# jpedro1992/gym-loadbalancing

Measured on AMD Instinct MI355X. Metric: env-steps/sec (whole node) at 1M envs, 1/2/4/8 GPUs; % HBM roofline, higher is better.
Workload: dtype f64

## Files before the change

### gym-loadbalancing_amd/csrc/lbk8s_lean.h

```cpp
#pragma once

#include "lbk8s_rollout.h"

namespace lbk {

typedef __amdgpu_buffer_rsrc_t Rsrc;
typedef uint32_t u32x2 __attribute__((ext_vector_type(2)));
typedef uint32_t u32x4 __attribute__((ext_vector_type(4)));

__device__ __forceinline__ Rsrc rsrc_of(const void* base) {
    return __builtin_amdgcn_make_buffer_rsrc(const_cast<void*>(base), (short)0, -1, 0x00020000);
}
constexpr int BUF_NT = 2;

#define LB_GUARD_S(...) asm volatile("" : "+s"(__VA_ARGS__))
#define LB_GUARD_V(...) asm volatile("" : "+v"(__VA_ARGS__))

__device__ __forceinline__ double buf_ld_f64(Rsrc r, uint32_t off) {
    return __builtin_bit_cast(double, __builtin_amdgcn_raw_buffer_load_b64(r, off, 0, 0));
}
__device__ __forceinline__ uint4 buf_ld_u128(Rsrc r, uint32_t off) {
    const u32x4 v = __builtin_amdgcn_raw_buffer_load_b128(r, off, 0, 0);
    return make_uint4(v.x, v.y, v.z, v.w);
}
template <int AUX>
__device__ __forceinline__ void buf_st_f4(float4 v, Rsrc r, uint32_t voff) {
    const u32x4 d{__float_as_uint(v.x), __float_as_uint(v.y), __float_as_uint(v.z), __float_as_uint(v.w)};
    __builtin_amdgcn_raw_buffer_store_b128(d, r, voff, 0, AUX);
}

__device__ __forceinline__ U4 draw_o(const Params& p, int64_t env, uint32_t episode, uint32_t slot, uint32_t dom) {
    uint32_t k0 = p.key0, k1 = p.key1;
    LB_GUARD_S(k0);
    LB_GUARD_S(k1);
    const uint64_t gid = (uint64_t)(p.env_id_offset + env);
    uint32_t c0 = (uint32_t)gid, hi = (uint32_t)(gid >> 32) << 8;
    LB_GUARD_V(c0);
    LB_GUARD_V(hi);
    return philox(c0, episode, slot, dom | hi, k0, k1);
}
__device__ __forceinline__ void draw2_o(const Params& p, int64_t env, uint32_t episode, uint32_t slot, uint32_t dom_a,
                                        uint32_t dom_b, U4& a, U4& b) {
    uint32_t k0 = p.key0, k1 = p.key1;
    LB_GUARD_S(k0);
    LB_GUARD_S(k1);
    const uint64_t gid = (uint64_t)(p.env_id_offset + env);
    uint32_t c0 = (uint32_t)gid, hi = (uint32_t)(gid >> 32) << 8;
    LB_GUARD_V(c0);
    LB_GUARD_V(hi);
    uint32_t a0 = c0, a1 = episode, a2 = slot, a3 = dom_a | hi;
    uint32_t b0 = c0, b1 = episode, b2 = slot, b3 = dom_b | hi;
#pragma unroll
    for (int i = 0; i < LB_PHILOX_ROUNDS; ++i) {
        const uint64_t pa0 = (uint64_t)0xD2511F53u * a0, pa1 = (uint64_t)0xCD9E8D57u * a2;
        const uint64_t pb0 = (uint64_t)0xD2511F53u * b0, pb1 = (uint64_t)0xCD9E8D57u * b2;
        const uint32_t na0 = (uint32_t)(pa1 >> 32) ^ a1 ^ k0, na2 = (uint32_t)(pa0 >> 32) ^ a3 ^ k1;
        const uint32_t nb0 = (uint32_t)(pb1 >> 32) ^ b1 ^ k0, nb2 = (uint32_t)(pb0 >> 32) ^ b3 ^ k1;
        a0 = na0; a1 = (uint32_t)pa1; a2 = na2; a3 = (uint32_t)pa0;
        b0 = nb0; b1 = (uint32_t)pb1; b2 = nb2; b3 = (uint32_t)pb0;
        k0 += 0x9E3779B9u;
        k1 += 0xBB67AE85u;
    }
    a = {a0, a1, a2, a3};
    b = {b0, b1, b2, b3};
}

template <int KIND>
__device__ __forceinline__ int lean_policy(const Params& p, int64_t env, const TEnv& tv, const uint32_t (&em)[TPE_E],
                                           const uint32_t (&ed)[TPE_E]) {
    if constexpr (KIND == LB_POLICY_RANDOM) {
        const U4 w = draw_o(p, env, (uint32_t)(tv.acc3 >> 32), (uint32_t)tv.s.step, D_ACT);
        return (int)bounded(w.x, (uint32_t)p.A);
    }
    return tpe_policy<KIND>(p, env, tv, em, ed);
}

__device__ __forceinline__ int topo_bf(uint64_t topo, int a, int b) {
    const int i = a < b ? a : b, j = a < b ? b : a;
    const int val = (int)((topo >> (9 * ((i * (7 - i)) / 2 + j - i - 1))) & 0x1FF);
    return a == b ? 1 : val;
}

struct LPrepL {
    uint32_t arz;
    uint32_t jm;
    double sel_lat, sel_cpu, next_lat, next_cpu, arr;
    float dt;
};

template <int ET, int RT, int RF>
__device__ __forceinline__ double lean_apply_l(const Params& p, const LPrepL& pr, LEnv& v,
                                               const uint32_t (&em)[TPE_E], uint32_t (&ed)[TPE_E], uint32_t* me) {
    constexpr int E = ET;
    const int rf = RF >= 0 ? RF : p.reward_fn;
    const int a = (int)(pr.arz & 0xFFu);
    const bool accept = a < E, reject = a == E;
    const int ai = accept ? a : 0;
    if (!((v.s1 >> S1_RD) & 1)) v.s1 |= 1u << S1_BAD;
    const int oA = (int)((pr.arz >> 14) & 7u);
    const int jA = (int)(pr.jm & 0x3FFu), Mn = (int)((pr.jm >> 10) & 0x3FFu), MA = (int)(pr.jm >> 20);
    const int jn = jA < CMAX ? jA + 1 : CMAX;
    double reward;
    if (accept) {
        int cnt = 0;
#pragma unroll
        for (int e = 0; e < TPE_E; ++e)
            if (e < E && e != ai && ed_j(ed[e]) <= jA) ++cnt;
        const int rz = (int)((v.s1 >> S1_RZ) & 3), zA = (int)((pr.arz >> 17) & 3u);
        const int tl = topo_bf(v.topo, rz, zA);
        const uint32_t gnum = (uint32_t)(v.acc2 >> 32) + (uint32_t)(2 * (2 * cnt - (E - 1)));
        v.acc2 = ((uint64_t)gnum << 32) | (uint32_t)((uint32_t)v.acc2 + (uint32_t)tl);
        v.acc3 += (uint64_t)node_cost((int)((pr.arz >> 19) & 7u));
        v.s0 += 1u << 16;
        if (rz == zA) v.s1 += 1;
        xsum_add(v.sum_lat, v.sum_cpu, v.sum_hi, pr.sel_lat, pr.sel_cpu, tl, rz != zA);
        const uint32_t edA_new = ((oA == ai ? (uint32_t)Mn : (uint32_t)MA) << 20) |
                                 ((uint32_t)Mn << 10) | (uint32_t)jn;
#pragma unroll
        for (int e = 0; e < TPE_E; ++e) {
            const uint32_t edo = e == oA ? (ed[e] & ~(0x3FFu << 20)) | ((uint32_t)Mn << 20) : ed[e];
            ed[e] = e == ai ? edA_new : edo;
        }
        img_sel(me, ai, (float)pr.next_cpu, (float)pr.next_lat);
        v.s1 &= ~(1u << S1_PEN);
        reward = rf == LB_REWARD_NAIVE ? 1.0 : accept_reward(p, pr.sel_lat, tl, pr.sel_cpu, v.acc2, (int)(v.s0 >> 16));
        v.last_r = reward;
    } else if (reject) {
        v.s1 |= 1u << S1_PEN;
        reward = rf == LB_REWARD_LATENCY ? -1000.0 : -1.0;
        v.last_r = reward;
    } else {
        reward = rf == LB_REWARD_NAIVE ? (((v.s1 >> S1_PEN) & 1) ? -1.0 : 1.0) : v.last_r;
    }
    v.total += reward;
    v.dt = pr.dt;
    v.t = pr.arr;
    v.s1 = (v.s1 & ~((3u << S1_RZ) | (7u << S1_THR))) | (((pr.arz >> 12) & 3u) << S1_RZ) |
           (((pr.arz >> 8) & 7u) << S1_THR);
    img_request(me, v, em, E);
    return reward;
}

constexpr uint32_t LREC_LAT0 = 96;
constexpr uint32_t LREC_ACC = 12;
__device__ __forceinline__ float4 u4f(double a, uint64_t b) {
    const uint64_t x = (uint64_t)__double_as_longlong(a);
    return make_float4(__uint_as_float((uint32_t)x), __uint_as_float((uint32_t)(x >> 32)), __uint_as_float((uint32_t)b),
                       __uint_as_float((uint32_t)(b >> 32)));
}
__device__ __forceinline__ float4 u4f(uint64_t a, uint64_t b) {
    return make_float4(__uint_as_float((uint32_t)a), __uint_as_float((uint32_t)(a >> 32)), __uint_as_float((uint32_t)b),
                       __uint_as_float((uint32_t)(b >> 32)));
}

template <int W>
__device__ __forceinline__ void lean_write_record(const Params& p, int64_t env, uint32_t episode, int lane) {
    static_assert(W == 8, "eight lanes per record (the node packing covers nodes < 24 = 3 x 8)");
    uint64_t zc = 0, nz0 = 0, nz1 = 0;
    uint32_t hp01 = 0, hp2 = 0;
    for (int w = 0; w < p.NZW; ++w) {
        uint64_t word = 0;
        int j = 0;
        for (int n = 32 * w + lane; n < 32 * (w + 1) && n < p.N; n += W, ++j) {
            int ty, zo, cpu;
            node_draw<false>(p, env, episode, n, ty, zo, cpu);
            zc += (uint64_t)node_cpu_int(ty) << (16 * zo);
            word |= (uint64_t)zo << (2 * (n & 31));
            const uint32_t hp = (uint32_t)ty | ((uint32_t)zo << 3) | ((uint32_t)cpu << 5);
            if (w == 0 && j == 0) hp01 |= hp;
            if (w == 0 && j == 1) hp01 |= hp << 16;
            if (w == 0 && j == 2) hp2 = hp;
        }
        word = slice_or64<W>(word);
        if (w == 0) nz0 = word;
        if (w == 1) nz1 = word;
    }
    zc = slice_sum64<W>(zc);
    double lat0 = 0.0;
    int node = 0;
    if (lane < p.E) {
        const U4 d = draw(p, env, episode, (uint32_t)lane, D_EP);
        lat0 = 1.0 + 99.0 * u53(d.x, d.y);
        node = (int)bounded(d.z, 24);
    }
    int owner = lane;
    for (int e2 = 0; e2 < p.E; ++e2) {
        const int nd2 = (int)shfl_u32<W>((uint32_t)node, e2);
        if (nd2 == node && e2 < owner) owner = e2;
    }
    const uint32_t ha = shfl_u32<W>(hp01, node & 7), hb = shfl_u32<W>(hp2, node & 7);
    const uint32_t hp = (node >> 3) == 0 ? (ha & 0xFFFFu) : (node >> 3) == 1 ? (ha >> 16) : hb;
    uint32_t* out = reinterpret_cast<uint32_t*>(p.rec + env * (RO_REC_BYTES / 16));
    if (lane < p.E) {
        const int ty = (int)(hp & 7u), zo = (int)((hp >> 3) & 3u), cpu = (int)((hp >> 5) & 0x7Fu);
        const uint64_t lb = (uint64_t)__double_as_longlong(lat0);
        *reinterpret_cast<uint2*>(out + 24 + 2 * lane) = make_uint2((uint32_t)lb, (uint32_t)(lb >> 32));
        out[lane] = em_pack(zo, owner, ty, cpu, node);
    }
    const int role = lane;
    const U4 w = draw(p, env, episode, role == 4 ? 1u : 0u,
                      role == 2 ? D_REQ_I : (role == 3 || role == 4) ? D_TOPO : D_REQ_X);
    const double e = role == 1 ? std_exp(w.z, w.w) : std_exp(w.x, w.y);
    const double x1 = p.inv_rate * shfl_f64<W>(e, 0), x2 = p.call * shfl_f64<W>(e, 1);
    const int r = (int)bounded(shfl_u32<W>(w.x, 2), 7), n = (int)bounded(shfl_u32<W>(w.y, 2), (uint32_t)p.N);
    const uint32_t a0 = shfl_u32<W>(w.x, 3), a1 = shfl_u32<W>(w.y, 3), a2 = shfl_u32<W>(w.z, 3),
                   a3 = shfl_u32<W>(w.w, 3), b0 = shfl_u32<W>(w.x, 4), b1 = shfl_u32<W>(w.y, 4);
    if (lane == 0) {
        const uint64_t topo = (uint64_t)(1 + bounded(a0, 499)) | ((uint64_t)(1 + bounded(a1, 499)) << 9) |
                              ((uint64_t)(1 + bounded(a2, 499)) << 18) | ((uint64_t)(1 + bounded(a3, 499)) << 27) |
                              ((uint64_t)(1 + bounded(b0, 499)) << 36) | ((uint64_t)(1 + bounded(b1, 499)) << 45);
        const int rz = (int)(((n < 32 ? nz0 : nz1) >> (2 * (n & 31))) & 3);
        const uint64_t wd[6] = {topo, zc, nz0, nz1, (uint64_t)__double_as_longlong(x1),
                                (uint64_t)__double_as_longlong(x2)};
#pragma unroll
        for (int j = 0; j < 6; ++j)
            *reinterpret_cast<uint2*>(out + 8 + 2 * j) = make_uint2((uint32_t)wd[j], (uint32_t)(wd[j] >> 32));
        out[20] = (uint32_t)((r + 6) % 7) | ((uint32_t)rz << 8);
    }
}

template <int ET, int RT, int NG>
__device__ __forceinline__ void lean_restart_group(const Params& p, const LDims<ET, RT>& d, uint32_t* wimg,
                                                   uint64_t grp, int lane, bool mine, LEnv& v,
                                                   uint32_t (&em)[TPE_E], uint32_t (&ed)[TPE_E], uint32_t* me) {
    if (mine) {
        const uint4* q = reinterpret_cast<const uint4*>(me);
        const uint4 s0 = q[2], s1 = q[3], s2 = q[4];
        const uint32_t s3 = me[20];
        v.topo = (uint64_t)s0.x | ((uint64_t)s0.y << 32);
        v.zcap = (uint64_t)s0.z | ((uint64_t)s0.w << 32);
        v.nz0 = (uint64_t)s1.x | ((uint64_t)s1.y << 32);
        v.nz1 = (uint64_t)s1.z | ((uint64_t)s1.w << 32);
        const uint32_t episode = (uint32_t)(v.acc3 >> 32) + 1;
        v.acc3 = (uint64_t)episode << 32;
        v.acc2 = 0;
        v.sum_lat = 0;
        v.sum_cpu = 0;
        v.sum_hi = 0;
        v.total = 0.0;
        v.last_r = p.init_last_r;
        v.s0 = 0;
        v.s1 = (v.s1 & (1u << S1_BAD)) | (1u << S1_RD) | ((s3 & 7u) << S1_THR) | (((s3 >> 8) & 3u) << S1_RZ);
        const double x1 = __longlong_as_double((long long)((uint64_t)s2.x | ((uint64_t)s2.y << 32)));
        const double x2 = __longlong_as_double((long long)((uint64_t)s2.z | ((uint64_t)s2.w << 32)));
        const double arrival = v.t + x1;
        const double departure = arrival + x2;
        v.dt = (float)(departure - arrival);
        v.t = arrival;
    }
    const int e = lane & 7, g = lane >> 3;
    int el = -1;
    {
        uint64_t m = grp;
#pragma unroll
        for (int i = 0; i < NG; ++i) {
            const int b = m ? (int)__builtin_ctzll(m) : -1;
            if (g == i) el = b;
            m &= m - 1;
        }
    }
    const bool helper = el >= 0 && e < ET;
    uint32_t* ri = wimg + (el < 0 ? 0 : el) * IMG_W;
    uint32_t mw = 0, l0lo = 0, l0hi = 0, zlo = 0, zhi = 0;
    if (helper) {
        mw = ri[e];
        l0lo = ri[24 + 2 * e];
        l0hi = ri[25 + 2 * e];
        zlo = ri[10];
        zhi = ri[11];
    }
    wave_lds_sync();
    if (helper) {
        const double l0 = __longlong_as_double((long long)((uint64_t)l0lo | ((uint64_t)l0hi << 32)));
        const int z = em_zone(mw);
        const uint64_t zcap = (uint64_t)zlo | ((uint64_t)zhi << 32);
        *reinterpret_cast<uint4*>(ri + 4 * e) =
            make_uint4(img_zc(z, zcap_val(zcap, z)), 0u, __float_as_uint((float)em_c0(mw)), __float_as_uint((float)l0));
        ri[32 + e] = lem_make(mw, l0);
    }
    wave_lds_sync();
    if (mine) {
        const uint4 a = *reinterpret_cast<const uint4*>(me + 32), b = *reinterpret_cast<const uint4*>(me + 36);
        const uint32_t lw[8] = {a.x, a.y, a.z, a.w, b.x, b.y, b.z, b.w};
#pragma unroll
        for (int i = 0; i < TPE_E; ++i) {
            em[i] = i < ET ? lw[i] : 0u;
            ed[i] = 0u;
        }
        *reinterpret_cast<uint4*>(me + 4 * d.E) = make_uint4(IMG_ZC_REJECT, F32_M1, F32_M1, F32_M1);
        img_request(me, v, em, d.E);
    }
}

template <int NJ>
__device__ __forceinline__ int rec_fetch_env(uint64_t m, int lane, int& chunk) {
    static_assert(NJ <= 6, "64 lanes: 6 records of 10 chunks");
    const int i = lane / 10;
    chunk = lane - 10 * i;
    int el = -1;
#pragma unroll
    for (int j = 0; j < NJ; ++j) {
        const int b = m ? (int)__builtin_ctzll(m) : -1;
        if (i == j) el = b;
        m &= m - 1;
    }
    return el;
}
constexpr int REC_FETCH_MAX = 6;

struct Acc {
    double total;
    uint64_t acc2, acc3, sum_lat, sum_cpu;
    uint32_t sum_hi, s0, s1;
};
template <int ET>
__device__ __forceinline__ void stats_row_lds(uint32_t* me, const Acc& a) {
    static_assert(LB_ST_RETURN == 0 && LB_ST_LENGTH == 1 && LB_ST_ACCEPTED == 2 && LB_ST_SUM_LATENCY == 3 &&
                      LB_ST_SUM_TOPOLOGY == 4 && LB_ST_SUM_TOPOLOGY_UPDATED == 5 && LB_ST_SUM_COST == 6 &&
                      LB_ST_SUM_CPU == 7 && LB_ST_INTRA == 8 && LB_ST_INTER == 9 && LB_ST_GINI == 10 &&
                      LB_ST_EPISODE == 11 && LB_ST_SUM_LATENCY_REM == 12 && LB_ST_SUM_CPU_REM == 13 &&
                      LB_ST_SUM_TOPOLOGY_UPDATED_D == 14 && LB_ST_K == 16,
                  "ep_stats column order");
    const Scal s = sc_unpack((uint64_t)a.s0 | ((uint64_t)a.s1 << 32));
    const uint32_t sum_topo = (uint32_t)a.acc2;
    auto put = [&](int i, double x, double y) {
        const uint64_t lo = (uint64_t)__double_as_longlong(x), hi = (uint64_t)__double_as_longlong(y);
        *reinterpret_cast<uint4*>(me + 4 * i) = make_uint4((uint32_t)lo, (uint32_t)(lo >> 32), (uint32_t)hi, (uint32_t)(hi >> 32));
    };
    double ls, lr, cs, cr;
    put(0, a.total, (double)s.step);
    xsum_pair(a.sum_lat, a.sum_hi & 0x7Fu, ls, lr);
    put(1, (double)s.acc, ls);
    put(2, (double)sum_topo, (double)s.intra + 1.7 * (double)(sum_topo - (uint32_t)s.intra));
    xsum_pair(a.sum_cpu, (a.sum_hi >> XH_CPU) & 0x1Fu, cs, cr);
    put(3, (double)(uint32_t)a.acc3, cs);
    put(4, (double)s.intra, (double)(s.acc - s.intra));
    put(5, gini_of(a.acc2, s.acc, ET), (double)(uint32_t)(a.acc3 >> 32));
    put(6, lr, cr);
    put(7, (double)((int32_t)a.sum_hi >> XH_D), 0.0);
}
__device__ __forceinline__ int nth_env8(uint64_t m, int i) {
    int el = -1;
#pragma unroll
    for (int j = 0; j < 8; ++j) {
        const int b = m ? (int)__builtin_ctzll(m) : -1;
        if (i == j) el = b;
        m &= m - 1;
    }
    return el;
}
__device__ __forceinline__ u32x4 lds_u4(const uint32_t* a) {
    const uint4 q = *reinterpret_cast<const uint4*>(a);
    return u32x4{q.x, q.y, q.z, q.w};
}

template <int P>
__device__ __forceinline__ int term_group_env(uint64_t m, int lane) {
    constexpr int G = 64 / P;
    const int g = lane / P;
    int el = -1;
#pragma unroll
    for (int i = 0; i < G; ++i) {
        const int b = m ? (int)__builtin_ctzll(m) : -1;
        if (g == i) el = b;
        m &= m - 1;
    }
    return el;
}
template <int P>
__device__ __forceinline__ uint64_t drop_low(uint64_t m) {
#pragma unroll
    for (int i = 0; i < 64 / P; ++i) m &= m - 1;
    return m;
}
__device__ __forceinline__ float4 term_piece(const uint32_t* wimg, int el, int pc) {
    const char* base = reinterpret_cast<const char*>(wimg) + el * (IMG_W * 4);
    const uint4 A = *reinterpret_cast<const uint4*>(base + 16 * (pc >> 1));
    const uint4 S = *reinterpret_cast<const uint4*>(base + 4 * IMG_S);
    return img_piece(A, S, (pc & 1) != 0);
}

template <int P>
__device__ __forceinline__ float4 lean_piece(const uint32_t* wimg, int lane, int it, bool h) {
    constexpr uint32_t MAG = (65536u + P - 1) / P;
    static_assert(P % 2 == 0 && 64u * P * (MAG * P - 65536u) < 65536u, "piece / P by multiply, exact below 64 P");
    const uint32_t e = ((uint32_t)lane * MAG + (uint32_t)it * (64u * MAG)) >> 16;
    const char* b = reinterpret_cast<const char*>(wimg);
    const uint4 A = *reinterpret_cast<const uint4*>(b + e * (uint32_t)(IMG_W * 4 - 8 * P) + 16u * (uint32_t)(lane >> 1) +
                                                    512u * (uint32_t)it);
    const uint4 S = *reinterpret_cast<const uint4*>(b + e * (uint32_t)(IMG_W * 4) + 4u * IMG_S);
    return img_piece(A, S, h);
}

#ifdef LB_TIMELINE
#include "../../tools/diag/lbk8s_lean_timeline.h"
#else
#define LB_LTL(k, i) ((void)0)
#define LB_LTL_HDR(slot) ((void)0)
#define LB_LTL_HWID() ((void)0)
#endif

constexpr int LEAN_NB = 64;

constexpr uint32_t SD_BASE = 3 * 64 * 4, SD_BUF = 64 * 20, SD_X2 = 64 * 8, SD_W = 64 * 16;
__device__ __forceinline__ double* sd_x1(uint32_t* sst, int b) {
    return reinterpret_cast<double*>(reinterpret_cast<char*>(sst) + SD_BASE + b * SD_BUF);
}
__device__ __forceinline__ double* sd_x2(uint32_t* sst, int b) { return sd_x1(sst, b) + 64; }
__device__ __forceinline__ uint32_t* sd_w(uint32_t* sst, int b) {
    return reinterpret_cast<uint32_t*>(reinterpret_cast<char*>(sst) + SD_BASE + b * SD_BUF + SD_W);
}
template <int KIND>
__device__ __forceinline__ void split_draws(const Params& p, int64_t env, uint32_t ep, uint32_t cs, uint32_t* sst,
                                            int b, int lane) {
    uint32_t a = 0;
    if constexpr (KIND == LB_POLICY_RANDOM) a = bounded(draw_o(p, env, ep, cs, D_ACT).x, (uint32_t)p.A);
    U4 wx, wi;
    draw2_o(p, env, ep, cs + 1, D_REQ_X, D_REQ_I, wx, wi);
    sd_x1(sst, b)[lane] = p.inv_rate * std_exp(wx.x, wx.y);
    sd_x2(sst, b)[lane] = p.call * std_exp(wx.z, wx.w);
    sd_w(sst, b)[lane] = a | (bounded(wi.x, 7) << 8) | (bounded(wi.y, (uint32_t)p.N) << 16);
}

template <int P, bool ACT, int CW, int KIND>
__device__ __forceinline__ void lean_copier(const Params& p, int K, int32_t* act_out, uint32_t (*simg)[64 * IMG_W],
                                            uint32_t* sst, int64_t env0) {
    const int lane = threadIdx.x & 63;
    const bool h = (lane & 1) != 0;
    uint32_t cs = 0, cep = 0;
#pragma unroll
    for (int c = 0; c < CW; ++c) {
        const int64_t env = env0 + 64 * c + lane;
        const uint64_t sc = p.sc[env], acc3 = p.acc3[env];
        cs = (uint32_t)(sc & 0xFFFF);
        cep = (uint32_t)(acc3 >> 32);
        const int to_done = p.L - (int)(sc & 0xFFFF);
        uint64_t mm = __ballot(to_done >= 1 && to_done <= K);
        const uint32_t epi = (uint32_t)(acc3 >> 32) + 1;
        const int g = lane / RS_W, gl = lane % RS_W;
        while (mm) {
            const int el = nth_env8(mm, g);
            const uint32_t ep = (uint32_t)__shfl((int)epi, el < 0 ? 0 : el);
            if (el >= 0) lean_write_record<RS_W>(p, env0 + 64 * c + el, ep, gl);
#pragma unroll
            for (int j = 0; j < 8; ++j) mm &= mm - 1;
        }
    }
    split_draws<KIND>(p, env0 + lane, cep, cs, sst, 0, lane);
    asm volatile("s_waitcnt vmcnt(0)" ::: "memory");
    block_lds_sync();
    for (int k = 0; k < K; ++k) {
        if (++cs == (uint32_t)p.L) {
            cs = 0;
            ++cep;
        }
        if (k + 1 < K) split_draws<KIND>(p, env0 + lane, cep, cs, sst, (k + 1) & 1, lane);
        block_lds_sync();
        float4 v[CW][P];
        uint32_t rw[CW], dn[CW], ac[CW];
#pragma unroll
        for (int c = 0; c < CW; ++c) {
#pragma unroll
            for (int it = 0; it < P; ++it) v[c][it] = lean_piece<P>(simg[c], lane, it, h);
            rw[c] = sst[192 * c + lane];
            dn[c] = sst[192 * c + 64 + lane];
            ac[c] = ACT ? sst[192 * c + 128 + lane] : 0u;
        }
        block_lds_sync();
        const Rsrc out = rsrc_of(p.obs + (int64_t)k * p.B * (P / 2) * 8);
        const Rsrc rwo = rsrc_of(p.reward + (int64_t)k * p.B), dno = rsrc_of(p.done + (int64_t)k * p.B);
#pragma unroll
        for (int c = 0; c < CW; ++c) {
            const uint32_t envi = (uint32_t)(env0 + 64 * c + lane);
            const uint32_t obs_wave = (uint32_t)((env0 + 64 * c) * P * 16);
#pragma unroll
            for (int it = 0; it < P; ++it)
                buf_st_f4<BUF_NT>(v[c][it], out, (uint32_t)lane * 16u + obs_wave + 1024u * (uint32_t)it);
            __builtin_amdgcn_raw_buffer_store_b32(rw[c], rwo, envi * 4u, 0, BUF_NT);
            __builtin_amdgcn_raw_buffer_store_b8((uint8_t)dn[c], dno, envi, 0, BUF_NT);
            if (ACT) __builtin_amdgcn_raw_buffer_store_b32(ac[c], rsrc_of(act_out + (int64_t)k * p.B), envi * 4u, 0, 0);
        }
    }
}

template <int KIND, int ET, int RT, int NZW, bool NAIVE, bool ACT, int CW>
__device__ __forceinline__ void lean_body(Params p, int K, int32_t* act_out, uint32_t (*simg)[64 * IMG_W],
                                          uint32_t* sstage) {
    static_assert(CW == 0 || CW == 1, "one env wave per copy wave (two: the copy wave's registers for both blocks spilled)");
    constexpr bool SPLIT = CW > 0;
    constexpr int NB = SPLIT ? 64 * (CW + 1) : LEAN_NB, NW = SPLIT ? CW : NB / 64, P = 2 * RT, GT = 64 / P;
    constexpr int FAST = GT < REC_FETCH_MAX ? GT : REC_FETCH_MAX;
    static_assert(ET >= 1 && ET <= TPE_E && (RT == ET || RT == ET + 1), "compile-time geometry");
    (void)NW;
    const LDims<ET, RT> d(p);
    const int lane = threadIdx.x & 63, wv = threadIdx.x >> 6;
    const int64_t blk = blockIdx.x;
    if constexpr (SPLIT) {
        if (wv == CW) {
            lean_copier<P, ACT, CW, KIND>(p, K, act_out, simg, sstage, blk * 64 * CW);
            return;
        }
    }
    uint32_t* wimg = simg[wv];
    uint32_t* me = wimg + lane * IMG_W;
    const int64_t env0 = blk * (SPLIT ? 64 * CW : NB) + __builtin_amdgcn_readfirstlane(threadIdx.x & ~63);
    if (env0 >= p.B) return;
    LB_LTL_HDR(2);
    LB_LTL_HWID();
    const int64_t env = env0 + lane;
    const uint32_t envi = (uint32_t)env;
    const Rsrc blob = rsrc_of(p.lat_lut);
    const uint32_t rec_off = (uint32_t)(reinterpret_cast<const char*>(p.rec) - reinterpret_cast<const char*>(p.lat_lut));
    const uint32_t cpu0 = (uint32_t)(reinterpret_cast<const char*>(p.cpu_lut) - reinterpret_cast<const char*>(p.lat_lut));

    LEnv v;
    uint32_t em[TPE_E], ed[TPE_E];
    double l0s[TPE_E];
    {
        const uint64_t sc = p.sc[env];
        v.acc3 = p.acc3[env];
        v.s0 = (uint32_t)sc;
        v.s1 = (uint32_t)(sc >> 32);
#pragma unroll
        for (int e = 0; e < TPE_E; ++e) {
            em[e] = 0u;
            ed[e] = 0u;
            l0s[e] = 0.0;
            if (e < ET) {
                const int64_t i = (int64_t)e * p.B + env;
                l0s[e] = p.lat0[i];
                em[e] = p.emeta[i];
                ed[e] = p.edyn[i];
            }
        }
        v.t = p.t[env];
        v.zcap = p.zcap[env];
        v.acc2 = p.acc2[env];
        v.topo = p.topo[env];
        v.nz0 = p.nzone[env];
        v.nz1 = NZW > 1 && p.NZW > 1 ? p.nzone[p.B + env] : 0;
        v.sum_lat = p.sum_lat[env];
        v.sum_cpu = p.sum_cpu[env];
        v.sum_hi = p.sum_hi[env];
        v.total = p.total[env];
        v.last_r = NAIVE ? 0.0 : p.last_r[env];
        v.dt = 0.f;
    }

    if constexpr (!SPLIT) {
        const int to_done = p.L - (int)(v.s0 & 0xFFFF);
        const bool fin = to_done >= 1 && to_done <= K;
        const uint64_t fm = __ballot(fin);
        if (fin) {
            uint32_t* it = wimg + 2 * __popcll(fm & ((1ull << lane) - 1));
            it[0] = (uint32_t)lane;
            it[1] = (uint32_t)(v.acc3 >> 32) + 1;
        }
        wave_lds_sync();
        const int nf = __popcll(fm), g = lane / RS_W, gl = lane % RS_W;
        for (int r0 = 0; r0 < nf; r0 += 64 / RS_W) {
            const int i = r0 + g;
            if (i < nf) lean_write_record<RS_W>(p, env0 + (int64_t)wimg[2 * i], wimg[2 * i + 1], gl);
        }
        asm volatile("s_waitcnt vmcnt(0) lgkmcnt(0)" ::: "memory");
    }
    LB_LTL_HDR(4);

    {
        float olat[TPE_E], ocpu[TPE_E];
#pragma unroll
        for (int e = 0; e < TPE_E; ++e) {
            olat[e] = 0.f;
            ocpu[e] = 0.f;
            if (e < ET) {
                const uint32_t m = em[e];
                em[e] = lem_make(m, l0s[e]);
                olat[e] = (float)lat_of(p, l0s[e], ed[e]);
                ocpu[e] = (float)cpu_of(p, m, ed[e]);
            }
        }
        img_endpoints(me, d, em, v.zcap, olat, ocpu);
    }

    __builtin_amdgcn_s_waitcnt(0xF70);
    LB_LTL_HDR(5);
    bool new_episode = false;
    uint32_t l0off = (uint32_t)(reinterpret_cast<const char*>(p.lat0) - reinterpret_cast<const char*>(p.lat_lut)) +
                     envi * 8u;
    uint32_t l0step = (uint32_t)p.B * 8u;
    const uint32_t obs_wave = (uint32_t)(env0 * P * 16);

    uint4 qn = make_uint4(0u, 0u, 0u, 0u);
    auto fetch_next = [&](int steps_done) {
        const uint64_t mn = __ballot((int)(steps_done + 1) == p.L);
        int chunk, ln = lane;
        LB_GUARD_V(ln);
        const int el = rec_fetch_env<FAST>(mn, ln, chunk);
        const uint32_t w0 = rec_off + (uint32_t)env0 * RO_REC_BYTES;
        qn = buf_ld_u128(blob, el >= 0 ? w0 + (uint32_t)el * RO_REC_BYTES + 16u * chunk : w0);
    };

    LPrepL pr;
    auto prep = [&](const int j, auto&& between) {
        (void)j;
        LPrepL r;
        TEnv tv;
        tv.topo = v.topo;
        tv.zcap = v.zcap;
        tv.acc3 = v.acc3;
        tv.s.rz = (int)((v.s1 >> S1_RZ) & 3);
        const int step = (int)(v.s0 & 0xFFFF);
        tv.s.step = step;
        const uint32_t dw = SPLIT ? sd_w(sstage, j & 1)[lane] : 0u;
        const int a = SPLIT && KIND == LB_POLICY_RANDOM ? (int)(dw & 0xFFu) : lean_policy<KIND>(p, env, tv, em, ed);
        const bool accept = a < ET;
        const int ai = accept ? a : 0;
        const uint32_t emA = pick8(em, ai), edA = pick8(ed, ai);
        const int oA = em_owner(emA);
        const uint32_t edO = pick8(ed, oA);
        const int jA = ed_j(edA);
        const int Mn = ed_M(edO) < CMAX ? ed_M(edO) + 1 : CMAX;
        const int jn = jA < CMAX ? jA + 1 : CMAX;
        const int k0A = lem_k0(emA), c0A = em_c0(emA);
        r.sel_lat = buf_ld_f64(blob, jA == 0 ? l0off + (uint32_t)ai * l0step : (uint32_t)(jA * LAT_ROWS + k0A) * 8u);
        r.sel_cpu = buf_ld_f64(blob, cpu0 + (uint32_t)(ed_m(edA) * CPU_ROWS + c0A) * 8u);
        r.next_lat = buf_ld_f64(blob, (uint32_t)(jn * LAT_ROWS + k0A) * 8u);
        r.next_cpu = buf_ld_f64(blob, cpu0 + (uint32_t)(Mn * CPU_ROWS + c0A) * 8u);
        fetch_next(step);
        asm volatile("" ::: "memory");
        between(0);
        asm volatile("" ::: "memory");
        double x1, x2;
        int rr, n;
        if constexpr (SPLIT) {
            x1 = sd_x1(sstage, j & 1)[lane];
            x2 = sd_x2(sstage, j & 1)[lane];
            rr = (int)((dw >> 8) & 0xFFu);
            n = (int)(dw >> 16);
        } else {
        const uint32_t episode = (uint32_t)(v.acc3 >> 32), slot = (uint32_t)(step + 1);
        U4 wx, wi;
        draw2_o(p, env, episode, slot, D_REQ_X, D_REQ_I, wx, wi);
        asm volatile("" ::"v"(wx.x), "v"(wx.y), "v"(wx.z), "v"(wx.w), "v"(wi.x), "v"(wi.y) : "memory");
        between(1);
        asm volatile("" ::: "memory");
        x1 = p.inv_rate * std_exp(wx.x, wx.y);
        asm volatile("" ::"v"(x1) : "memory");
        between(2);
        asm volatile("" ::: "memory");
        x2 = p.call * std_exp(wx.z, wx.w);
        rr = (int)bounded(wi.x, 7);
        n = (int)bounded(wi.y, (uint32_t)p.N);
        }
        r.arr = v.t + x1;
        r.dt = (float)((r.arr + x2) - r.arr);
        asm volatile("" ::"v"(r.arr), "v"(r.dt) : "memory");
        between(3);
        asm volatile("" ::: "memory");
        const uint64_t word = (NZW > 1 && n >= 32) ? v.nz1 : v.nz0;
        const uint32_t rz = (uint32_t)((word >> (2 * (n & 31))) & 3);
        r.arz = (uint32_t)a | ((uint32_t)((rr + 6) % 7) << 8) | (rz << 12) | ((uint32_t)oA << 14) |
                ((uint32_t)em_zone(emA) << 17) | ((uint32_t)em_type(emA) << 19);
        r.jm = (uint32_t)jA | ((uint32_t)Mn << 10) | ((uint32_t)ed_M(edA) << 20);
        asm volatile("" ::"v"(r.arz) : "memory");
        between(4);
        asm volatile("" ::: "memory");
        between(5);
        return r;
    };
    if constexpr (SPLIT) block_lds_sync();
    pr = prep(0, [](int) {});
    asm volatile("" : "+v"(pr.sel_lat), "+v"(pr.sel_cpu), "+v"(pr.next_lat), "+v"(pr.next_cpu), "+v"(qn.x), "+v"(qn.y),
                 "+v"(qn.z), "+v"(qn.w));

    auto iter = [&](const int k) {
        LB_LTL(k, 0);
        {
            const int pl = 3 - (4 * k) / K;
            if (pl >= 3) __builtin_amdgcn_s_setprio(3);
            else if (pl == 2) __builtin_amdgcn_s_setprio(2);
            else if (pl == 1) __builtin_amdgcn_s_setprio(1);
            else __builtin_amdgcn_s_setprio(0);
        }
        const int a_k = (int)(pr.arz & 0xFFu);
        v.s0 += 1;
        const bool done = (int)(v.s0 & 0xFFFF) == p.L;
        const double reward = lean_apply_l<ET, RT, NAIVE ? (int)LB_REWARD_NAIVE : -1>(p, pr, v, em, ed, me);
        const uint64_t m = __ballot(done);
        LB_LTL(k, 1);
        if (m) {
            wave_lds_sync();
            const int pc = lane % P;
            bool pre = __popcll(m) <= FAST;
            for (uint64_t mm = m; mm;) {
                uint64_t grp = mm;
#pragma unroll
                for (int j = 0; j < FAST; ++j) mm &= mm - 1;
                grp &= ~mm;
                const int tel = term_group_env<P>(grp, lane);
                if (tel >= 0)
                    buf_st_f4<BUF_NT>(term_piece(wimg, tel, pc), rsrc_of(p.term_obs),
                                      (uint32_t)((env0 + tel) * P + pc) * 16u);
                const bool mine = done && ((grp >> lane) & 1);
                int chunk;
                const int rl = rec_fetch_env<FAST>(grp, lane, chunk);
                uint4* dst = reinterpret_cast<uint4*>(wimg + rl * IMG_W + 4 * chunk);
                wave_lds_sync();
                if (pre) {
                    if (rl >= 0) *dst = qn;
                } else {
                    if (rl >= 0) *dst = buf_ld_u128(blob, rec_off + (uint32_t)(env0 + rl) * RO_REC_BYTES + 16u * chunk);
                }
                if (mine) {
                    const uint32_t o = rec_off + envi * RO_REC_BYTES + 4u * LREC_ACC;
                    buf_st_f4<0>(u4f(v.total, v.acc2), blob, o);
                    buf_st_f4<0>(u4f(v.sum_lat, v.sum_cpu), blob, o + 16u);
                    buf_st_f4<0>(make_float4(__uint_as_float((uint32_t)v.acc3), __uint_as_float(v.sum_hi),
                                             __uint_as_float(v.s0), __uint_as_float(v.s1)),
                                 blob, o + 32u);
                }
                wave_lds_sync();
                lean_restart_group<ET, RT, FAST>(p, d, wimg, grp, lane, mine, v, em, ed, me);
                if (mine) {
                    new_episode = true;
                    l0off = rec_off + envi * RO_REC_BYTES + LREC_LAT0;
                    l0step = 8u;
                }
                pre = false;
            }
        }
        LB_LTL(k, 2);
        if constexpr (SPLIT) {
            sstage[192 * wv + lane] = __float_as_uint((float)reward);
            sstage[192 * wv + 64 + lane] = done ? 1u : 0u;
            if (ACT) sstage[192 * wv + 128 + lane] = (uint32_t)a_k;
            block_lds_sync();
            LB_LTL(k, 3);
            if (k + 1 < K) {
                pr = prep(k + 1, [](int) {});
                asm volatile("" : "+v"(pr.sel_lat), "+v"(pr.sel_cpu), "+v"(pr.next_lat), "+v"(pr.next_cpu),
                             "+v"(qn.x), "+v"(qn.y), "+v"(qn.z), "+v"(qn.w));
            }
            LB_LTL(k, 4);
            block_lds_sync();
            LB_LTL(k, 5);
            return;
        }
        const Rsrc out = rsrc_of(p.obs + k * (int64_t)p.B * RT * 8);
        const Rsrc rw = rsrc_of(p.reward + (int64_t)k * p.B), dn = rsrc_of(p.done + (int64_t)k * p.B);
        wave_lds_sync();
        const bool h = (lane & 1) != 0;
        auto stores = [&](int stage) {
            if (stage == 0) {
                LB_LTL(k, 3);
                if (ACT) __builtin_amdgcn_raw_buffer_store_b32((uint32_t)a_k, rsrc_of(act_out + (int64_t)k * p.B),
                                                               envi * 4u, 0, 0);
                __builtin_amdgcn_raw_buffer_store_b32(__float_as_uint((float)reward), rw, envi * 4u, 0, BUF_NT);
                __builtin_amdgcn_raw_buffer_store_b8((uint8_t)done, dn, envi, 0, BUF_NT);
            }
            constexpr int per = (P + PREP_STAGES - 1) / PREP_STAGES;
            uint32_t so = obs_wave + 1024u * (uint32_t)(stage * per);
            LB_GUARD_S(so);
            int ln = lane;
            LB_GUARD_V(ln);
#pragma unroll
            for (int it = stage * per; it < (stage + 1) * per && it < P; ++it) {
                buf_st_f4<BUF_NT>(lean_piece<P>(wimg, ln, it, h), out,
                                  (uint32_t)ln * 16u + so + 1024u * (uint32_t)(it - stage * per));
            }
        };
        if (k + 1 < K) {
            pr = prep(k + 1, stores);
            LB_LTL(k, 4);
            asm volatile("" : "+v"(pr.sel_lat), "+v"(pr.sel_cpu), "+v"(pr.next_lat), "+v"(pr.next_cpu), "+v"(qn.x),
                         "+v"(qn.y), "+v"(qn.z), "+v"(qn.w));
            LB_LTL(k, 5);
        } else {
            for (int s = 0; s < PREP_STAGES; ++s) stores(s);
        }
        wave_lds_sync();
    };
    LB_LTL_HDR(0);
    if (K > 0) iter(0);
    for (int k = 1; k < K; ++k) iter(k);
    LB_LTL_HDR(1);
    {
        const uint64_t endm = __ballot(new_episode);
        if (endm) {
            if (new_episode) {
                const uint32_t o = rec_off + envi * RO_REC_BYTES + 4u * LREC_ACC;
                const uint4 q0 = buf_ld_u128(blob, o), q1 = buf_ld_u128(blob, o + 16u), q2 = buf_ld_u128(blob, o + 32u);
                auto u64 = [](uint32_t lo, uint32_t hi) { return (uint64_t)lo | ((uint64_t)hi << 32); };
                const uint64_t acc3 = ((uint64_t)((uint32_t)(v.acc3 >> 32) - 1u) << 32) | q2.x;
                stats_row_lds<ET>(me, Acc{__longlong_as_double((long long)u64(q0.x, q0.y)), u64(q0.z, q0.w), acc3,
                                          u64(q1.x, q1.y), u64(q1.z, q1.w), q2.y, q2.z, q2.w});
            }
            wave_lds_sync();
#pragma unroll
            for (int i = 0; i < 8; ++i) {
                const int el = 8 * i + (lane >> 3), c = lane & 7;
                if ((endm >> el) & 1)
                    __builtin_amdgcn_raw_buffer_store_b128(lds_u4(wimg + el * IMG_W + 4 * c), rsrc_of(p.ep_stats),
                                                           (uint32_t)(env0 + el) * (uint32_t)(8 * LB_ST_K) + 16u * (uint32_t)c,
                                                           0, 0);
            }
        }
    }
    int64_t ew = env;
    asm volatile("" : "+v"(ew));
#pragma unroll
    for (int e = 0; e < TPE_E; ++e)
        if (e < ET) p.edyn[(int64_t)e * p.B + ew] = ed[e];
    if (new_episode) {
        const uint32_t* w = reinterpret_cast<const uint32_t*>(p.rec + ew * (RO_REC_BYTES / 16));
#pragma unroll
        for (int e = 0; e < TPE_E; ++e) {
            if (e >= ET) continue;
            const int64_t i = (int64_t)e * p.B + ew;
            p.lat0[i] = __longlong_as_double((long long)((uint64_t)w[24 + 2 * e] | ((uint64_t)w[25 + 2 * e] << 32)));
            p.emeta[i] = w[e];
        }
        p.topo[ew] = v.topo;
        p.zcap[ew] = (uint64_t)w[10] | ((uint64_t)w[11] << 32);
        p.nzone[ew] = v.nz0;
        if (NZW > 1 && p.NZW > 1) p.nzone[p.B + ew] = v.nz1;
    }
    p.t[ew] = v.t;
    p.sc[ew] = (uint64_t)v.s0 | ((uint64_t)v.s1 << 32);
    p.acc2[ew] = v.acc2;
    p.acc3[ew] = v.acc3;
    p.sum_lat[ew] = v.sum_lat;
    p.sum_cpu[ew] = v.sum_cpu;
    p.sum_hi[ew] = v.sum_hi;
    p.total[ew] = v.total;
    if (!NAIVE) p.last_r[ew] = v.last_r;
    LB_LTL_HDR(3);
}

template <int KIND, int ET, int RT, int NZW, bool NAIVE, bool ACT>
__global__ __launch_bounds__(LEAN_NB, 4) void k_rollout_lean(Params p, int K, int32_t* act_out) {
    __shared__ __attribute__((aligned(16))) uint32_t simg[LEAN_NB / 64][64 * IMG_W];
    lean_body<KIND, ET, RT, NZW, NAIVE, ACT, 0>(p, K, act_out, simg, nullptr);
}
template <int KIND, int ET, int RT, int NZW, bool NAIVE, bool ACT, int CW>
__global__ __launch_bounds__(64 * (CW + 1), 4) void k_rollout_lean_split(Params p, int K,
                                                                                       int32_t* act_out) {
    __shared__ __attribute__((aligned(16))) uint32_t simg[CW][64 * IMG_W];
    __shared__ __attribute__((aligned(16))) uint32_t sstage[CW * 3 * 64 + 2 * SD_BUF / 4];
    lean_body<KIND, ET, RT, NZW, NAIVE, ACT, CW>(p, K, act_out, simg, sstage);
}

}
```

Before: 20.15 billion.

## Precompute restart record layout so each env restarts itself without wave-cooperative LDS passes

The per-env reset record is repacked so the writer precomputes the zone-capacity halves, the packed episode metadata words and the node ids. Each terminating env can then rebuild its own observation image from the record, instead of a grouped, helper-lane restart with two extra wave syncs. A single-terminating-env fast path avoids the group loop. In the split kernel, accumulator stats are staged in LDS rather than round-tripped through global memory. These changes add LDS footprint and more complex record packing. SA_W indexing by lane may collide across consumer waves, which is a risk.

```diff
diff --git a/gym-loadbalancing_amd/csrc/lbk8s_lean.h b/gym-loadbalancing_amd/csrc/lbk8s_lean.h
--- a/gym-loadbalancing_amd/csrc/lbk8s_lean.h
+++ b/gym-loadbalancing_amd/csrc/lbk8s_lean.h
@@ -142,7 +142,7 @@
 }
 
 constexpr uint32_t LREC_LAT0 = 96;
-constexpr uint32_t LREC_ACC = 12;
+__device__ __forceinline__ constexpr uint32_t lrec_acc(int c) { return c < 2 ? 16u * (uint32_t)(c + 1) : 64u; }
 __device__ __forceinline__ float4 u4f(double a, uint64_t b) {
     const uint64_t x = (uint64_t)__double_as_longlong(a);
     return make_float4(__uint_as_float((uint32_t)x), __uint_as_float((uint32_t)(x >> 32)), __uint_as_float((uint32_t)b),
@@ -188,14 +188,16 @@
         const int nd2 = (int)shfl_u32<W>((uint32_t)node, e2);
         if (nd2 == node && e2 < owner) owner = e2;
     }
+    const uint64_t nds = slice_or64<W>((uint64_t)(uint32_t)node << (5 * (lane & 3) + 32 * (lane >> 2)));
+    const uint32_t nd03 = (uint32_t)nds, nd47 = (uint32_t)(nds >> 32);
     const uint32_t ha = shfl_u32<W>(hp01, node & 7), hb = shfl_u32<W>(hp2, node & 7);
     const uint32_t hp = (node >> 3) == 0 ? (ha & 0xFFFFu) : (node >> 3) == 1 ? (ha >> 16) : hb;
     uint32_t* out = reinterpret_cast<uint32_t*>(p.rec + env * (RO_REC_BYTES / 16));
     if (lane < p.E) {
         const int ty = (int)(hp & 7u), zo = (int)((hp >> 3) & 3u), cpu = (int)((hp >> 5) & 0x7Fu);
         const uint64_t lb = (uint64_t)__double_as_longlong(lat0);
-        *reinterpret_cast<uint2*>(out + 24 + 2 * lane) = make_uint2((uint32_t)lb, (uint32_t)(lb >> 32));
-        out[lane] = em_pack(zo, owner, ty, cpu, node);
+        out[16 + lane] = lem_make(em_pack(zo, owner, ty, cpu, node), lat0);
+        *reinterpret_cast<uint2*>(out + LREC_LAT0 / 4 + 2 * lane) = make_uint2((uint32_t)lb, (uint32_t)(lb >> 32));
     }
     const int role = lane;
     const U4 w = draw(p, env, episode, role == 4 ? 1u : 0u,
@@ -214,19 +216,25 @@
                                 (uint64_t)__double_as_longlong(x2)};
 #pragma unroll
         for (int j = 0; j < 6; ++j)
-            *reinterpret_cast<uint2*>(out + 8 + 2 * j) = make_uint2((uint32_t)wd[j], (uint32_t)(wd[j] >> 32));
-        out[20] = (uint32_t)((r + 6) % 7) | ((uint32_t)rz << 8);
-    }
-}
-
-template <int ET, int RT, int NG>
-__device__ __forceinline__ void lean_restart_group(const Params& p, const LDims<ET, RT>& d, uint32_t* wimg,
-                                                   uint64_t grp, int lane, bool mine, LEnv& v,
-                                                   uint32_t (&em)[TPE_E], uint32_t (&ed)[TPE_E], uint32_t* me) {
-    if (mine) {
-        const uint4* q = reinterpret_cast<const uint4*>(me);
-        const uint4 s0 = q[2], s1 = q[3], s2 = q[4];
-        const uint32_t s3 = me[20];
+            *reinterpret_cast<uint2*>(out + 2 * j) = make_uint2((uint32_t)wd[j], (uint32_t)(wd[j] >> 32));
+        out[12] = (uint32_t)((r + 6) % 7) | ((uint32_t)rz << 8) | (nd03 << 12);
+        uint64_t zcf = 0;
+#pragma unroll
+        for (int z = 0; z < 4; ++z) zcf |= (uint64_t)(img_zc(z, zcap_val(zc, z)) >> 16) << (16 * z);
+        *reinterpret_cast<uint2*>(out + 14) = make_uint2((uint32_t)zcf, (uint32_t)(zcf >> 32));
+        out[13] = nd47;
+    }
+}
+
+template <int ET>
+__device__ __forceinline__ void lean_restart_self(const Params& p, int E, LEnv& v, uint32_t (&em)[TPE_E],
+                                                  uint32_t (&ed)[TPE_E], uint32_t* me) {
+    uint4* q = reinterpret_cast<uint4*>(me);
+    uint64_t zcf;
+    {
+        const uint4 s0 = q[0], s1 = q[1], s2 = q[2], s4 = q[3];
+        const uint32_t s3 = s4.x;
+        zcf = (uint64_t)s4.z | ((uint64_t)s4.w << 32);
         v.topo = (uint64_t)s0.x | ((uint64_t)s0.y << 32);
         v.zcap = (uint64_t)s0.z | ((uint64_t)s0.w << 32);
         v.nz0 = (uint64_t)s1.x | ((uint64_t)s1.y << 32);
@@ -248,48 +256,32 @@
         v.dt = (float)(departure - arrival);
         v.t = arrival;
     }
-    const int e = lane & 7, g = lane >> 3;
-    int el = -1;
     {
-        uint64_t m = grp;
-#pragma unroll
-        for (int i = 0; i < NG; ++i) {
-            const int b = m ? (int)__builtin_ctzll(m) : -1;
-            if (g == i) el = b;
-            m &= m - 1;
-        }
-    }
-    const bool helper = el >= 0 && e < ET;
-    uint32_t* ri = wimg + (el < 0 ? 0 : el) * IMG_W;
-    uint32_t mw = 0, l0lo = 0, l0hi = 0, zlo = 0, zhi = 0;
-    if (helper) {
-        mw = ri[e];
-        l0lo = ri[24 + 2 * e];
-        l0hi = ri[25 + 2 * e];
-        zlo = ri[10];
-        zhi = ri[11];
-    }
-    wave_lds_sync();
-    if (helper) {
-        const double l0 = __longlong_as_double((long long)((uint64_t)l0lo | ((uint64_t)l0hi << 32)));
-        const int z = em_zone(mw);
-        const uint64_t zcap = (uint64_t)zlo | ((uint64_t)zhi << 32);
-        *reinterpret_cast<uint4*>(ri + 4 * e) =
-            make_uint4(img_zc(z, zcap_val(zcap, z)), 0u, __float_as_uint((float)em_c0(mw)), __float_as_uint((float)l0));
-        ri[32 + e] = lem_make(mw, l0);
-    }
-    wave_lds_sync();
-    if (mine) {
-        const uint4 a = *reinterpret_cast<const uint4*>(me + 32), b = *reinterpret_cast<const uint4*>(me + 36);
+        const uint4 a = q[4], b = q[5];
         const uint32_t lw[8] = {a.x, a.y, a.z, a.w, b.x, b.y, b.z, b.w};
 #pragma unroll
         for (int i = 0; i < TPE_E; ++i) {
             em[i] = i < ET ? lw[i] : 0u;
             ed[i] = 0u;
         }
-        *reinterpret_cast<uint4*>(me + 4 * d.E) = make_uint4(IMG_ZC_REJECT, F32_M1, F32_M1, F32_M1);
-        img_request(me, v, em, d.E);
-    }
+    }
+#pragma unroll
+    for (int h = 0; h < 4; ++h) {
+        if (2 * h >= ET) continue;
+        const uint4 l = q[6 + h];
+        const uint32_t lo[2] = {l.x, l.z}, hi[2] = {l.y, l.w};
+#pragma unroll
+        for (int i = 0; i < 2; ++i) {
+            const int e = 2 * h + i;
+            if (e >= ET) continue;
+            const double l0 = __longlong_as_double((long long)((uint64_t)lo[i] | ((uint64_t)hi[i] << 32)));
+            const uint32_t z = em[e] & 3u;
+            const uint32_t zc = (uint32_t)__builtin_bit_cast(uint16_t, (_Float16)(int)z) | ((uint32_t)(zcf >> (16u * z)) << 16);
+            q[e] = make_uint4(zc, 0u, __float_as_uint((float)em_c0(em[e])), __float_as_uint((float)l0));
+        }
+    }
+    *reinterpret_cast<uint4*>(me + 4 * E) = make_uint4(IMG_ZC_REJECT, F32_M1, F32_M1, F32_M1);
+    img_request(me, v, em, E);
 }
 
 template <int NJ>
@@ -403,6 +395,7 @@
 constexpr int LEAN_NB = 64;
 
 constexpr uint32_t SD_BASE = 3 * 64 * 4, SD_BUF = 64 * 20, SD_X2 = 64 * 8, SD_W = 64 * 16;
+constexpr uint32_t SA_W = (SD_BASE + 2 * SD_BUF) / 4, SA_WORDS = 64 * 12;
 __device__ __forceinline__ double* sd_x1(uint32_t* sst, int b) {
     return reinterpret_cast<double*>(reinterpret_cast<char*>(sst) + SD_BASE + b * SD_BUF);
 }
@@ -690,43 +683,60 @@
         LB_LTL(k, 1);
         if (m) {
             wave_lds_sync();
-            const int pc = lane % P;
-            bool pre = __popcll(m) <= FAST;
-            for (uint64_t mm = m; mm;) {
-                uint64_t grp = mm;
-#pragma unroll
-                for (int j = 0; j < FAST; ++j) mm &= mm - 1;
-                grp &= ~mm;
-                const int tel = term_group_env<P>(grp, lane);
-                if (tel >= 0)
-                    buf_st_f4<BUF_NT>(term_piece(wimg, tel, pc), rsrc_of(p.term_obs),
-                                      (uint32_t)((env0 + tel) * P + pc) * 16u);
-                const bool mine = done && ((grp >> lane) & 1);
-                int chunk;
-                const int rl = rec_fetch_env<FAST>(grp, lane, chunk);
-                uint4* dst = reinterpret_cast<uint4*>(wimg + rl * IMG_W + 4 * chunk);
+            if (__popcll(m) == 1) {
+                const int el = (int)__builtin_ctzll(m);
+                if (lane < P)
+                    buf_st_f4<BUF_NT>(term_piece(wimg, el, lane), rsrc_of(p.term_obs),
+                                      (uint32_t)((env0 + el) * P + lane) * 16u);
                 wave_lds_sync();
-                if (pre) {
-                    if (rl >= 0) *dst = qn;
+                LB_LTL(k, 6);
+                if (lane < 10) *reinterpret_cast<uint4*>(wimg + el * IMG_W + 4 * lane) = qn;
+            } else {
+                const int pc = lane % P;
+                bool pre = __popcll(m) <= FAST;
+                for (uint64_t mm = m; mm;) {
+                    uint64_t grp = mm;
+#pragma unroll
+                    for (int j = 0; j < FAST; ++j) mm &= mm - 1;
+                    grp &= ~mm;
+                    const int tel = term_group_env<P>(grp, lane);
+                    if (tel >= 0)
+                        buf_st_f4<BUF_NT>(term_piece(wimg, tel, pc), rsrc_of(p.term_obs),
+                                          (uint32_t)((env0 + tel) * P + pc) * 16u);
+                    int chunk;
+                    const int rl = rec_fetch_env<FAST>(grp, lane, chunk);
+                    uint4* dst = reinterpret_cast<uint4*>(wimg + rl * IMG_W + 4 * chunk);
+                    wave_lds_sync();
+                    if (pre) {
+                        if (rl >= 0) *dst = qn;
+                    } else {
+                        if (rl >= 0) *dst = buf_ld_u128(blob, rec_off + (uint32_t)(env0 + rl) * RO_REC_BYTES + 16u * chunk);
+                    }
+                    pre = false;
+                }
+                LB_LTL(k, 6);
+            }
+            if (done) {
+                const float4 a0 = u4f(v.total, v.acc2), a1 = u4f(v.sum_lat, v.sum_cpu),
+                             a2 = make_float4(__uint_as_float((uint32_t)v.acc3), __uint_as_float(v.sum_hi),
+                                              __uint_as_float(v.s0), __uint_as_float(v.s1));
+                if constexpr (SPLIT) {
+                    float4* a = reinterpret_cast<float4*>(sstage + SA_W + 12 * lane);
+                    a[0] = a0, a[1] = a1, a[2] = a2;
                 } else {
-                    if (rl >= 0) *dst = buf_ld_u128(blob, rec_off + (uint32_t)(env0 + rl) * RO_REC_BYTES + 16u * chunk);
+                    const uint32_t o = rec_off + envi * RO_REC_BYTES;
+                    buf_st_f4<0>(a0, blob, o + lrec_acc(0));
+                    buf_st_f4<0>(a1, blob, o + lrec_acc(1));
+                    buf_st_f4<0>(a2, blob, o + lrec_acc(2));
                 }
-                if (mine) {
-                    const uint32_t o = rec_off + envi * RO_REC_BYTES + 4u * LREC_ACC;
-                    buf_st_f4<0>(u4f(v.total, v.acc2), blob, o);
-                    buf_st_f4<0>(u4f(v.sum_lat, v.sum_cpu), blob, o + 16u);
-                    buf_st_f4<0>(make_float4(__uint_as_float((uint32_t)v.acc3), __uint_as_float(v.sum_hi),
-                                             __uint_as_float(v.s0), __uint_as_float(v.s1)),
-                                 blob, o + 32u);
-                }
-                wave_lds_sync();
-                lean_restart_group<ET, RT, FAST>(p, d, wimg, grp, lane, mine, v, em, ed, me);
-                if (mine) {
-                    new_episode = true;
-                    l0off = rec_off + envi * RO_REC_BYTES + LREC_LAT0;
-                    l0step = 8u;
-                }
-                pre = false;
+            }
+            wave_lds_sync();
+            LB_LTL(k, 7);
+            if (done) {
+                lean_restart_self<ET>(p, d.E, v, em, ed, me);
+                new_episode = true;
+                l0off = rec_off + envi * RO_REC_BYTES + LREC_LAT0;
+                l0step = 8u;
             }
         }
         LB_LTL(k, 2);
@@ -788,8 +798,14 @@
         const uint64_t endm = __ballot(new_episode);
         if (endm) {
             if (new_episode) {
-                const uint32_t o = rec_off + envi * RO_REC_BYTES + 4u * LREC_ACC;
-                const uint4 q0 = buf_ld_u128(blob, o), q1 = buf_ld_u128(blob, o + 16u), q2 = buf_ld_u128(blob, o + 32u);
+                const uint32_t o = rec_off + envi * RO_REC_BYTES;
+                uint4 q0, q1, q2;
+                if constexpr (SPLIT) {
+                    const uint4* a = reinterpret_cast<const uint4*>(sstage + SA_W + 12 * lane);
+                    q0 = a[0], q1 = a[1], q2 = a[2];
+                } else {
+                    q0 = buf_ld_u128(blob, o + lrec_acc(0)), q1 = buf_ld_u128(blob, o + lrec_acc(1)), q2 = buf_ld_u128(blob, o + lrec_acc(2));
+                }
                 auto u64 = [](uint32_t lo, uint32_t hi) { return (uint64_t)lo | ((uint64_t)hi << 32); };
                 const uint64_t acc3 = ((uint64_t)((uint32_t)(v.acc3 >> 32) - 1u) << 32) | q2.x;
                 stats_row_lds<ET>(me, Acc{__longlong_as_double((long long)u64(q0.x, q0.y)), u64(q0.z, q0.w), acc3,
@@ -817,11 +833,13 @@
         for (int e = 0; e < TPE_E; ++e) {
             if (e >= ET) continue;
             const int64_t i = (int64_t)e * p.B + ew;
-            p.lat0[i] = __longlong_as_double((long long)((uint64_t)w[24 + 2 * e] | ((uint64_t)w[25 + 2 * e] << 32)));
-            p.emeta[i] = w[e];
+            p.lat0[i] = __longlong_as_double(
+                (long long)((uint64_t)w[LREC_LAT0 / 4 + 2 * e] | ((uint64_t)w[LREC_LAT0 / 4 + 1 + 2 * e] << 32)));
+            const uint32_t node = ((e < 4 ? w[12] >> (12 + 5 * e) : w[13] >> (5 * (e - 4)))) & 0x1Fu;
+            p.emeta[i] = (em[e] & 0xFFFFFu) | (node << 20);
         }
         p.topo[ew] = v.topo;
-        p.zcap[ew] = (uint64_t)w[10] | ((uint64_t)w[11] << 32);
+        p.zcap[ew] = (uint64_t)w[2] | ((uint64_t)w[3] << 32);
         p.nzone[ew] = v.nz0;
         if (NZW > 1 && p.NZW > 1) p.nzone[p.B + ew] = v.nz1;
     }
@@ -846,7 +864,7 @@
 __global__ __launch_bounds__(64 * (CW + 1), 4) void k_rollout_lean_split(Params p, int K,
                                                                                        int32_t* act_out) {
     __shared__ __attribute__((aligned(16))) uint32_t simg[CW][64 * IMG_W];
-    __shared__ __attribute__((aligned(16))) uint32_t sstage[CW * 3 * 64 + 2 * SD_BUF / 4];
+    __shared__ __attribute__((aligned(16))) uint32_t sstage[CW * 3 * 64 + 2 * SD_BUF / 4 + CW * SA_WORDS];
     lean_body<KIND, ET, RT, NZW, NAIVE, ACT, CW>(p, K, act_out, simg, sstage);
 }
 
```

Result: no change. 20.33 billion (median of 6 runs) (+0.9%).
